# OpenMined/PIR

Measured on AMD Instinct MI355X. Metric: PIR queries/sec (ms/query in ms_per_step), N=4096 DB=2^20 x 288B d=2, higher is better.
Workload: dtype u64; 1 GPU; N=4096, 2 RNS data primes (36,36 bit | special 37 bit), t=24 bit, DB=2^20 x 288B, d=2, dims=[162, 162], num_pt=26215, 64 queries/step (whole job), 16 in flight per GPU (BASELINE.json configs[2]); workers=16, dist_mode=single, exchange=none, parallelism=single GPU, database_copies_in_hbm=operand layout only (u64 staging released)

## Files before the change

### pir_amd/build.py

```python
from __future__ import annotations

import os
import subprocess
import sys

HERE = os.path.dirname(os.path.abspath(__file__))
CSRC = os.path.join(HERE, "csrc")
LIB = os.path.join(HERE, "libpirgpu.so")
SOURCES = ["kernels.hip", "scan_mfma.hip", "ctx.hip", "wire.cpp", "wire_codec.cpp",
           "ntt_ring32k.hip",
           "ctmult.hip",
           "ctmult_rowsum.hip",
           "ctmult_shared.hip"]
NTT_SOURCE = "ntt_kernels.hip"
NTT_LOGNS = [11, 12, 13, 14]
NTT_PACK_BYTES = [5, 6, 7]
HEADERS = ["device_params.h", "env_gate.h", "options.h", "kernels.h", "host_math.h", "wire.h", "wire_codec.h", "arith.h", "ntt_core.h", "ctmult.h", "ctmult_convert.h", "scan_mfma_body.inc", NTT_SOURCE, os.path.join("..", "..", "include", "pirgpu.h")]
HIPCC = os.environ.get("HIPCC", "/opt/rocm/bin/hipcc")
FLAGS = ["--offload-arch=gfx950", "-O3", "-std=c++17", "-fPIC", "-Wall", "-Wno-unused-function"] + \
    os.environ.get("PIRGPU_BUILD_DEFS", "").split()


def ntt_object(logn: int, pb: int) -> str:
    return "ntt_kernels_%d.o" % logn if pb == 5 else "ntt_kernels_%d_p%d.o" % (logn, pb)


def _stale() -> bool:
    if not os.path.exists(LIB):
        return True
    t = os.path.getmtime(LIB)
    for f in SOURCES + HEADERS + [os.path.basename(__file__)]:
        p = os.path.join(CSRC, f) if f != os.path.basename(__file__) else os.path.join(HERE, f)
        if os.path.exists(p) and os.path.getmtime(p) > t:
            return True
    return False


def build(force: bool = False, verbose: bool = False) -> str:
    if not force and not _stale():
        return LIB
    jobs = []
    for src in SOURCES:
# ... 50 lines not shown
```

### pir_amd/csrc/ctx.hip

```cpp
#include <hip/hip_runtime.h>
#include <ctype.h>
#include <stdint.h>
#include <stdio.h>
#include <stdlib.h>
#include <string.h>

#include <algorithm>
#include <atomic>
#include <functional>
#include <map>
#include <mutex>
#include <string>
#include <vector>

#include "../../include/pirgpu.h"
#include "ctmult.h"
#include "device_params.h"
#include "host_math.h"
#include "kernels.h"
#include "options.h"
#include "wire.h"

using namespace pirgpu;

// ... 38 lines not shown
  uint32_t keyset = 0;
  uint32_t table = 0;
  uint64_t *res_a = nullptr, *res_b = nullptr, *prod = nullptr, *dig = nullptr, *sv_ntt = nullptr;
  uint64_t* d_query = nullptr;
  uint32_t staged_nq = 0;
  const uint64_t* sv_cur = nullptr;
  const uint64_t* sv_rows = nullptr;
  std::vector<uint64_t*> lvl;
  uint64_t* last = nullptr;
  uint64_t* pt_buf = nullptr;
  uint64_t* scan_part = nullptr;
  uint64_t* up_scratch = nullptr;
  size_t up_scratch_words = 0;
  uint8_t* selp = nullptr;
  bool reply_valid = false;
  hipEvent_t ev_expanded = nullptr, ev_scanned = nullptr;
  hipEvent_t ev_done = nullptr;
  hipEvent_t ev_join = nullptr;
};

struct HeadSlot {
  uint64_t *res_a = nullptr, *res_b = nullptr, *dig = nullptr, *prod = nullptr;
  hipEvent_t ev_ready = nullptr;
  hipEvent_t ev_free = nullptr;
  bool in_use = false;
};

struct BatchLane {
  hipStream_t stream = nullptr;
  HeadSlot head[2];
  uint32_t head_next = 0;
  uint64_t *res_a = nullptr, *res_b = nullptr, *prod = nullptr, *dig = nullptr;
  uint8_t* selp = nullptr;
  uint8_t* selp_runs = nullptr;
  hipEvent_t ev_scanned = nullptr;
  hipEvent_t ev_join = nullptr;
  std::vector<uint64_t*> lvl;
  uint64_t* last = nullptr;
  uint64_t* pt_buf = nullptr;
  uint64_t* scan_part = nullptr;
  uint64_t* up_scratch = nullptr;
  size_t up_scratch_words = 0;
};

struct Stage {
  hipStream_t stream;
  uint64_t* const* lvl;
  uint64_t* pt_buf;
  uint32_t n;
  MfmaPtrs sel;
  bool local_rows;
  uint64_t** up_scratch = nullptr;
  size_t* up_scratch_words = nullptr;
  bool sel_f64 = false;
  uint64_t* last = nullptr;
  bool rows_inverted = false;
  uint32_t ksets[kMaxMfmaQueries] = {};
};

struct CtmScratch {
  uint64_t* buf = nullptr;
  size_t words = 0;
  uint64_t* selc = nullptr;
  size_t selc_words = 0;
  uint64_t* selb = nullptr;
};
// ... 85 lines not shown
  std::map<uint32_t, uint16_t*> gperm;

  bool ws_ready = false;
  std::vector<Worker> workers;
  std::vector<uint64_t> lvl_rows;
  std::vector<uint64_t> lvl_cts;
  uint64_t m_max = 1;
  uint64_t pt_words = 0;
  BatchSet sets[kBatchSets];
  BatchSet& bs();
  uint32_t n_active = 1;
  uint32_t upper_blocks = 0;
  uint32_t upper_blocks_batch = 0;
  uint32_t scan_wgs_batch = 0;
  int64_t slots_scan_wgs = -1;
  bool slots_gather_ntt = false, slots_blk_major = false;
  bool tables_one_launch = false;
  int64_t ctm_rowsum_splits = 0;
  bool in_batch = false;
  uint32_t scan_nsplit = 1, scan_cps = 0, scan_rows = 0, scan_cols = 0;
  uint32_t scan_rpt = 0, scan_block = 0;
  bool scan_limb = false;
  uint32_t mq_nq = 4, mq_rows = 1;
  bool mq_single = false;
  uint32_t mq_single_rows = 4;
  bool mq_single_limb = false;
  uint64_t scan_npt = 0;
  bool mfma_on = false;
  MfmaGeom mg{};
  uint32_t mfma_nq = 0;
  bool mfma_single = false;
  bool scan_f64_fold = false;
  bool scan_f64_fold_batch = false;
  bool split_upper = false;
  uint64_t split_upper_words = 0;
  bool loop_transforms = false;
  uint32_t loop_min_sources = 1024;
  uint32_t fuse_mac_nodes = 128;
  bool fuse_mac_combine = false;
  bool fuse_last_level = false;
  bool last_level_ntt = false;
  bool tree40 = false;
  bool c0_ntt = false;
  bool c0_ntt_split = false;
  bool want_sel_f64 = false;
  bool sel_f64 = false;
  bool pack40 = false;
  int pack_bytes = 5;
  uint8_t* d_dbp = nullptr;
  bool packed_valid = false;
  bool staging_released = false;
  bool streamed = false;
  uint64_t stream_bands = 1;
  uint64_t db_bytes = 0, dbp_alloc = 0, mem_scratch = 0, mem_peak = 0;
  std::vector<BatchLane> lanes;
  uint64_t groups_run = 0;
  hipStream_t head_stream = nullptr;
  uint32_t head_levels = 0;
  uint32_t head_mode = 0;
  hipEvent_t ev_head_tail = nullptr;
  hipStream_t copy_stream = nullptr;
  hipEvent_t ev_fetch[2] = {nullptr, nullptr};
  hipEvent_t ev_fork = nullptr;
  hipEvent_t ev_main_join = nullptr;

  bool ctm = false;
// ... 354 lines not shown
  if (c->logN >= 15) c->split_upper = true;
  c->split_upper_words = (uint64_t)opt_u32(c, OPT_SPLIT_UPPER_MB, 3072) * (1ull << 20) / 8;
  c->loop_transforms = opt_u32(c, OPT_LOOP_TRANSFORMS, 1) != 0 && c->mode != kNttInt;
  c->pack40 = opt_u32(c, OPT_PACK40, 1) != 0;
  {
    uint32_t bits = 0;
    for (uint32_t j = 0; j <= k; ++j) bits = std::max<uint32_t>(bits, 64 - (uint32_t)__builtin_clzll(c->hp.mod[j].q));
    const int need = bits <= 39 ? 5 : (bits <= 47 ? 6 : (bits <= 55 ? 7 : 8));
    int want = (int)opt_u32(c, OPT_PACK_BYTES, (uint32_t)need);
    if (want < need) want = need;
    if (c->mode == kNttInt && want != 5) want = 8;
    if (c->logN >= 15) want = 8;
    if (want > 7) c->pack40 = false;
    c->pack_bytes = c->pack40 ? want : 5;
    if (c->pack40 && c->pack_bytes == 7 && c->logN >= 14 && !opt_u32(c, OPT_TREE40_WIDE, 0)) c->tree40 = false;
    const NttOps* ops = ntt_ops_for(N, c->pack_bytes);
    if (ops != c->ops) {
      c->ops = ops;
      HIP_TRY(c->ops->configure(c->mode));
    }
  }
  bool wide_given = false;
  const int64_t wide = c->options.value(OPT_SCAN_MFMA_WIDE, 0, &wide_given);
  c->mg = mfma_geometry(c->hp, c->scan_rows, c->scan_cols, wide_given ? (int)(wide != 0) : -1,
                        opt_u32(c, OPT_SCAN_MFMA_TOP4, 1) != 0);
  c->mfma_on = opt_u32(c, OPT_SCAN_MFMA, 1) != 0 && d >= 2 && c->mg.L != 0 && c->scan_rows >= 8 && c->scan_npt > 0;
  if (c->slot_sharded && (!c->mfma_on || c->mg.nchunks != 1 || c->nslots % c->mg.NW))
    throw Fail{PIRGPU_INVALID_ARGUMENT, "a slot shard needs the int8-MFMA scan in one column chunk (d = 2, >= 8 rows, "
                                        "moduli below 2^55, at most 28 column groups)"};
  c->mfma_nq = std::max<uint32_t>(1, std::min<uint32_t>(opt_u32(c, OPT_SCAN_MFMA_NQ, kMaxMfmaQueries), kMaxMfmaQueries));
  c->mfma_single = opt_u32(c, OPT_SCAN_MFMA_SINGLE, c->mg.nchunks == 1 ? 1 : 0) != 0;
  c->scan_f64_fold = opt_u32(c, OPT_SCAN_F64_FOLD, c->mg.L >= 6 ? 1 : 0) != 0;
  c->scan_f64_fold_batch = opt_u32(c, OPT_SCAN_F64_FOLD_BATCH, 1) != 0;
  for (uint32_t j = 0; j < k; ++j) {
    c->scan_f64_fold = c->scan_f64_fold && (c->hp.mod[j].q >> 50) == 0;
    c->scan_f64_fold_batch = c->scan_f64_fold_batch && (c->hp.mod[j].q >> 50) == 0;
  }
  const uint64_t rem = c->dim_sum % N;
  c->sel_f64 = c->want_sel_f64 && c->mfma_on && c->mode != kNttInt && c->fuse_last_level && c->last_level_ntt &&
               !c->split_upper && c->dim_sum >= 2 && rem != 1 && !c->ctm;
  if (c->ctm) c->ctm_scratch_words = (uint64_t)std::max<int64_t>(1, c->options.value(OPT_CT_SCRATCH_MB, 256)) * (1ull << 20) / 8;
  c->ctm_shared_sel = c->ctm && c->options.value(OPT_CT_SHARED_SEL, ctm_shared_sel_default(c)) != 0;
  if (c->streamed && c->mfma_on) {
    const uint64_t mb = (uint64_t)std::max<int64_t>(0, c->options.value(OPT_DB_STREAM_MB, 256));
    c->stream_bands = std::min<uint64_t>(std::max<uint64_t>(1, (mb << 20) / stream_band_bytes(c)), 65535);
    c->mfma_single = true;
  }
}

void ensure_workspace(pirgpu_ctx* c) {
  if (c->ws_ready) return;
  const uint32_t N = c->N, k = c->k, d = c->d;

  const uint64_t m_max = std::min<uint64_t>(N, hm::next_power_two(std::max<uint32_t>(c->dim_sum, 1)));
  c->m_max = m_max;
  const uint64_t shard_pts = matrix_pts(c);
  if (d == 1) {
    c->scan_rows = c->planes;
    c->scan_cols = (uint32_t)(shard_pts / c->planes);
  } else {
    c->scan_cols = c->dims[d - 1];
    c->scan_rows = (uint32_t)ceil_div(shard_pts, c->scan_cols);
  }
  c->scan_npt = shard_pts;
  resolve_options(c);
  c->lvl_rows.assign(d, 0);
// ... 398 lines not shown
  const uint64_t words = (uint64_t)c->scan_rows * c->ctw;
  ensure_packed(c);
  uint64_t* const out = c->mg.nchunks > 1 ? part : out_base;
  const uint64_t out_qstride = c->mg.nchunks > 1 ? (uint64_t)c->mg.nchunks * words : words;
  if (!packed) {
    if (!selp) selp = c->dalloc<uint8_t>(c->mg.sel_bytes);
    HIP_TRY(launch_sel_pack(st, c->dp, c->mg, col_sel, n, selp, c->scan_cols, kN, sel_f64));
    packed = selp;
  }
  if (profiled) record(c, *profiled, PH_SCAN);
  const bool share = share_chip && !profiled && c->scan_wgs_batch;
  const uint32_t wgs = share ? c->scan_wgs_batch : 0;
  constexpr uint32_t kMaxBscan = 64;
  const bool timed = c->prof && !profiled && c->bscan_n < kMaxBscan;
  if (timed) {
    while (c->bscan_ev.size() < 2 * (size_t)(c->bscan_n + 1)) {
      hipEvent_t e;
      HIP_TRY(hipEventCreate(&e));
      c->bscan_ev.push_back(e);
    }
    HIP_TRY(hipEventRecord(c->bscan_ev[2 * c->bscan_n], st));
  }
  HIP_TRY(launch_scan_mfma(st, c->dp, c->mg, table_dbp(c, table), packed, out, out_qstride, n, c->scan_rows, kN, words, wgs,
                           n > 1 ? (c->scan_f64_fold || c->scan_f64_fold_batch) : c->scan_f64_fold));
  if (!profiled) ++c->options.counter(OPT_SCAN_LAUNCHES);
  if (timed) {
    HIP_TRY(hipEventRecord(c->bscan_ev[2 * c->bscan_n + 1], st));
    ++c->bscan_n;
    c->bscan_wgs = wgs;
    c->bscan_nq = n;
  }
  if (c->mg.nchunks > 1)
    HIP_TRY(launch_reduce_splits(st, c->dp, part, c->mg.nchunks, words, out_base, n, (uint64_t)c->mg.nchunks * words, words));
}

void scan_on_device(pirgpu_ctx* c, Worker& w) {
  const uint32_t N = c->N, k = c->k;
  const size_t ctw = c->ctw;
  refuse_slot_shard(c);
  if (!table_loaded(c, w.table))
    throw Fail{PIRGPU_FAILED_PRECONDITION, c->tables > 1 ? "table " + std::to_string(w.table) + " not fully loaded"
                                                         : std::string("database not fully loaded")};
  check_transparent(c, w.table);
  if (c->pt_end == c->pt_begin) return;
  if (c->mfma_on && c->mfma_single) {
    MfmaPtrs col{};
    col.p[0] = scan_selectors(c, w);
    scan_group_mfma(c, w.stream, w.selp, col, 1, scan_out(c, w), w.scan_part, &w, nullptr, false, false, w.table);
    return;
  }
  const uint64_t* sv_base = scan_selectors(c, w);
  uint64_t* base_out = scan_out(c, w);
  const uint64_t* db = table_db(c, w.table);
  if (c->mq_single && mq_usable(c)) {
    HIP_TRY(launch_scan_mq(w.stream, c->dp, N, k, db, &sv_base, &base_out, 1, c->scan_rows, c->scan_cols,
                           c->mq_single_rows, c->mq_single_limb && c->scan_limb));
    return;
  }
  uint64_t* scan_out = c->scan_nsplit > 1 ? w.scan_part : base_out;
  HIP_TRY(launch_scan(w.stream, c->dp, N, k, db, sv_base, scan_out, c->scan_rows, c->scan_cols, c->scan_npt,
                      c->scan_nsplit, c->scan_cps, c->scan_rpt, c->scan_block, c->scan_limb));
  if (c->scan_nsplit > 1)
    HIP_TRY(launch_reduce_splits(w.stream, c->dp, w.scan_part, c->scan_nsplit, (uint64_t)c->scan_rows * ctw,
                                 base_out));
}

// ... 2107 lines not shown
}

static void ensure_lanes(pirgpu_ctx* c, bool with_expansion_buffers) {
  const uint32_t N = c->N, k = c->k;
  if (c->lanes.empty()) {
    const uint32_t n_lanes = 2;
    c->lanes.resize(n_lanes);
    for (BatchLane& ln : c->lanes) {
      HIP_TRY(hipStreamCreateWithFlags(&ln.stream, hipStreamNonBlocking));
      HIP_TRY(hipEventCreateWithFlags(&ln.ev_scanned, hipEventDisableTiming));
    }
  }
  if (with_expansion_buffers && !c->lanes[0].res_a) {
    const uint64_t half = std::max<uint64_t>(c->m_max / 2, 1);
    for (BatchLane& ln : c->lanes) {
      ln.res_a = c->dalloc<uint64_t>((size_t)kMaxMfmaQueries * c->m_max * c->ctw);
      ln.res_b = c->dalloc<uint64_t>((size_t)kMaxMfmaQueries * c->m_max * c->ctw);
      ln.prod = c->dalloc<uint64_t>((size_t)kMaxMfmaQueries * half * 2 * (k + 1) * N);
      ln.dig = c->dalloc<uint64_t>((size_t)kMaxMfmaQueries * half * (k + 1) * k * N);
    }
  }
  if (c->mfma_on && c->lanes[0].lvl.empty()) {
    for (BatchLane& ln : c->lanes) {
      ln.lvl.assign(c->d, nullptr);
      for (uint32_t l = 0; l < c->d; ++l) ln.lvl[l] = c->dalloc<uint64_t>((size_t)kMaxMfmaQueries * c->lvl_cts[l] * c->ctw);
      if (c->rp) ln.last = c->dalloc<uint64_t>((size_t)kMaxMfmaQueries * c->lvl_cts[0] * c->ctw);
      if (c->pt_words) ln.pt_buf = c->dalloc<uint64_t>((size_t)kMaxMfmaQueries * c->pt_words);
      if (c->mg.nchunks > 1)
        ln.scan_part = c->dalloc<uint64_t>((size_t)kMaxMfmaQueries * c->mg.nchunks * std::max<uint32_t>(c->scan_rows, 1) * c->ctw);
    }
  }
}

static void ensure_head_slot(pirgpu_ctx* c, HeadSlot& hs) {
  if (hs.res_a) return;
  const uint32_t N = c->N, k = c->k;
  const uint64_t cts = ((uint64_t)1 << c->head_levels) * kMaxMfmaQueries;
  hs.res_a = c->dalloc<uint64_t>(cts * c->ctw);
  hs.res_b = c->dalloc<uint64_t>(cts * c->ctw);
  hs.prod = c->dalloc<uint64_t>(std::max<uint64_t>(cts / 2, 1) * 2 * (k + 1) * N);
  hs.dig = c->dalloc<uint64_t>(std::max<uint64_t>(cts / 2, 1) * (k + 1) * k * N);
  HIP_TRY(hipEventCreateWithFlags(&hs.ev_ready, hipEventDisableTiming));
  HIP_TRY(hipEventCreateWithFlags(&hs.ev_free, hipEventDisableTiming));
  if (!c->head_stream) {
    HIP_TRY(hipStreamCreateWithFlags(&c->head_stream, hipStreamNonBlocking));
    HIP_TRY(hipEventCreateWithFlags(&c->ev_head_tail, hipEventDisableTiming));
  }
}

static void expand_group_on_lane(pirgpu_ctx* c, BatchLane& ln, Worker* const* members, uint32_t B, uint32_t first,
                                 bool sel_f64 = false, uint64_t* sv_dst = nullptr, const uint32_t* qidx = nullptr) {
  const uint32_t N = c->N, k = c->k;
  const uint32_t nq = c->dim_sum / N + 1;
  const size_t ctw = c->ctw, qwords = (size_t)nq * ctw;
  uint64_t remaining = c->dim_sum, produced = 0;
  const bool use_head = nq == 1 && B > 1 && c->head_levels > 0 && (c->head_mode == 2 || (c->head_mode == 1 && c->bs().st_pieces > 0)) &&
                        hm::ceil_log2((uint32_t)std::min<uint64_t>(c->dim_sum, N)) >= c->head_levels + 2;
  const uint32_t ws_first = qidx ? 0 : first, ws_n = qidx ? c->bs().staged_count : B;
  if (!use_head) wait_staged(c, ln.stream, ws_first, ws_n);
  auto import_roots = [&](hipStream_t st, uint64_t* dst, uint32_t qc) {
    if (!qidx) {
      HIP_TRY(launch_tree_convert(st, c->dp, c->mode, c->bs().d_bquery + (size_t)first * qwords + (size_t)qc * ctw, dst,
                                  (uint64_t)B * ctw, true, ctw, qwords));
      return;
    }
    for (uint32_t q = 0; q < B; ++q)
// ... 103 lines not shown
}

static uint32_t lanes_in_use(pirgpu_ctx* c, uint32_t G) {
  const uint32_t W = std::max<uint32_t>(1, std::min<uint32_t>(c->n_active, (uint32_t)c->workers.size()));
  return std::max<uint32_t>(1, std::min<uint32_t>((uint32_t)c->lanes.size(), W / std::max<uint32_t>(G, 1)));
}

static void batch_run_mfma(pirgpu_ctx* c, uint32_t count, const uint64_t* ext_sv, const PackedInput* pk = nullptr,
                           const uint32_t* qtab = nullptr) {
  const size_t rwords = (size_t)c->reply_cts * c->rctw, svwords = (size_t)c->dim_sum * c->ctw;
  const uint32_t W = std::max<uint32_t>(1, std::min<uint32_t>(c->n_active, (uint32_t)c->workers.size()));
  const uint32_t G = std::min<uint32_t>(c->mfma_nq, W);
  TablePlan tp;
  if (qtab) tp = plan_table_runs(qtab, count, G);
  const uint32_t* order = qtab && !tp.identity ? tp.order.data() : nullptr;
  auto oq = [&](uint32_t pos) { return order ? order[pos] : pos; };
  auto tab = [&](uint32_t pos) { return qtab ? qtab[oq(pos)] : 0u; };
  std::vector<uint8_t> done(order ? count : 0, 0);
  uint32_t lead = 0;
  const uint32_t my_rows = c->se - c->sb;
  ensure_lanes(c, !ext_sv && !pk);
  const uint32_t nl = lanes_in_use(c, G);
  const uint32_t span = pk ? pk->per_rank : count;
  uint32_t n_groups = 0;
  for (uint32_t rank0 = 0; rank0 < count; rank0 += span) {
    const uint32_t in_span = std::min<uint32_t>(span, count - rank0);
    n_groups += (in_span + (pk ? (uint32_t)kMaxMfmaQueries : G) - 1) / (pk ? (uint32_t)kMaxMfmaQueries : G);
  }
  const bool share_chip = n_groups >= 2 && nl >= 2;
  const bool host_dl = c->bs().host_reply && (uint64_t)count * c->reply_cts <= c->bs().host_reply_cts;
  c->bs().host_reply_done = host_dl;
  c->bs().dl_end.clear();
  c->bs().dl_next = 0;
  for (uint32_t rank0 = 0; rank0 < count; rank0 += span) {
    const uint32_t step = pk ? (uint32_t)kMaxMfmaQueries : G;
    const uint32_t in_span = std::min<uint32_t>(span, count - rank0);
    for (uint32_t j0 = 0; j0 < in_span; j0 += step) {
      const uint32_t B = std::min<uint32_t>(step, in_span - j0);
      if (B > W) throw Fail{PIRGPU_FAILED_PRECONDITION, "packed groups need min(queries per rank, 8) workers (pirgpu_set_concurrency)"};
      const uint32_t li = (uint32_t)(c->groups_run++ % nl);
      BatchLane& ln = c->lanes[li];
      Worker* members[kMaxMfmaQueries];
      for (uint32_t q = 0; q < B; ++q) {
        members[q] = &c->workers[(li * G + q) % W];
        HIP_TRY(hipStreamWaitEvent(ln.stream, members[q]->ev_done, 0));
      }
      const uint32_t first = rank0 + j0;
      const uint8_t* packed = nullptr;
      uint64_t* lvl_ptrs[PIRGPU_MAX_DIMS];
      for (uint32_t l = 0; l < c->d; ++l) lvl_ptrs[l] = ln.lvl[l];
      const bool direct_reply = c->d >= 2 && !order;
      if (direct_reply) lvl_ptrs[0] = reply_base(c) + (size_t)first * rwords;
      Stage sg{ln.stream, lvl_ptrs, ln.pt_buf, B, MfmaPtrs{}, pk != nullptr, &ln.up_scratch, &ln.up_scratch_words};
      sg.last = ln.last;
      for (uint32_t q = 0; q < B; ++q)
        sg.ksets[q] = oq(first + q) < c->bs().batch_keysets.size() ? c->bs().batch_keysets[oq(first + q)] : 0;
      MfmaPtrs col{};
      if (pk) {
        const uint32_t groups_per_rank = (pk->per_rank + kMaxMfmaQueries - 1) / kMaxMfmaQueries;
        packed = pk->packed + ((size_t)(rank0 / pk->per_rank) * groups_per_rank + j0 / kMaxMfmaQueries) * c->mg.sel_bytes;
        for (uint32_t q = 0; q < B; ++q) sg.sel.p[q] = pk->rows + (size_t)(first + q) * my_rows * c->ctw;
      } else {
        if (!ext_sv) {
          expand_group_on_lane(c, ln, members, B, first, c->sel_f64, nullptr, order ? order + first : nullptr);
          sg.sel_f64 = c->sel_f64;
        }
        for (uint32_t q = 0; q < B; ++q) {
          const uint64_t* sv = ext_sv ? ext_sv + (size_t)oq(first + q) * svwords : members[q]->sv_ntt;
          sg.sel.p[q] = sv;
          col.p[q] = sv + (size_t)c->sv_off[c->d - 1] * c->ctw;
        }
      }
      uint32_t rb[kMaxMfmaQueries + 1], tabs[kMaxMfmaQueries], nr = 0;
      for (uint32_t q = 0; q < B; ++q)
        if (q == 0 || tab(first + q) != tab(first + q - 1)) {
          rb[nr] = q;
          tabs[nr++] = tab(first + q);
        }
      rb[nr] = B;
      if (nr == 1)
        scan_group_mfma(c, ln.stream, ln.selp, col, B, ln.lvl[c->d - 1], ln.scan_part, nullptr, packed, sg.sel_f64,
                        share_chip, tabs[0]);
      else
        scan_group_runs(c, ln, col, B, rb, nr, tabs, sg.sel_f64, share_chip);
      post_scan_stage(c, sg, nullptr);
      if (order) {
        for (uint32_t q = 0; q < B; ++q)
          HIP_TRY(hipMemcpyAsync(reply_base(c) + (size_t)oq(first + q) * rwords, ln.lvl[0] + (size_t)q * rwords, rwords * 8,
                                 hipMemcpyDeviceToDevice, ln.stream));
      } else if (!direct_reply)
        HIP_TRY(hipMemcpyAsync(reply_base(c) + (size_t)first * rwords, ln.lvl[0], (size_t)B * rwords * 8,
                               hipMemcpyDeviceToDevice, ln.stream));
      if (host_dl) {
        BatchSet& b = c->bs();
        const size_t gi = b.dl_end.size();
        while (gi >= b.dl_events.size()) {
          hipEvent_t e;
          HIP_TRY(hipEventCreateWithFlags(&e, hipEventDisableTiming));
          b.dl_events.push_back(e);
          HIP_TRY(hipEventCreateWithFlags(&e, hipEventDisableTiming));
          b.rd_events.push_back(e);
        }
        if (!c->copy_stream) HIP_TRY(hipStreamCreateWithFlags(&c->copy_stream, hipStreamNonBlocking));
        HIP_TRY(hipEventRecord(b.rd_events[gi], ln.stream));
        HIP_TRY(hipStreamWaitEvent(c->copy_stream, b.rd_events[gi], 0));
        if (order) {
          for (uint32_t q = 0; q < B; ++q) {
            const size_t at = (size_t)oq(first + q) * rwords;
            HIP_TRY(hipMemcpyAsync(b.host_reply + at, reply_base(c) + at, rwords * 8, hipMemcpyDeviceToHost, c->copy_stream));
            done[oq(first + q)] = 1;
          }
          while (lead < count && done[lead]) ++lead;
        } else {
          HIP_TRY(hipMemcpyAsync(b.host_reply + (size_t)first * rwords, reply_base(c) + (size_t)first * rwords,
                                 (size_t)B * rwords * 8, hipMemcpyDeviceToHost, c->copy_stream));
        }
        HIP_TRY(hipEventRecord(b.dl_events[gi], c->copy_stream));
        b.dl_end.push_back(order ? lead : first + B);
      }
      for (uint32_t q = 0; q < B; ++q) {
        HIP_TRY(hipEventRecord(members[q]->ev_done, ln.stream));
        members[q]->reply_valid = false;
      }
    }
  }
}

static void batch_run_impl_body(pirgpu_ctx* c, uint32_t count, const uint64_t* ext_sv);
static void batch_run_impl(pirgpu_ctx* c, uint32_t count, const uint64_t* ext_sv) {
  struct Flag {
    bool& f;
    explicit Flag(bool& x) : f(x) { f = true; }
    ~Flag() { f = false; }
  } flag(c->in_batch);
  batch_run_impl_body(c, count, ext_sv);
}
static void batch_run_impl_body(pirgpu_ctx* c, uint32_t count, const uint64_t* ext_sv) {
  refuse_slot_shard(c);
  c->bs().host_reply_done = false;
  const size_t rwords = (size_t)c->reply_cts * c->rctw;
  const size_t svwords = (size_t)c->dim_sum * c->ctw;
  const uint32_t W = std::max<uint32_t>(1, std::min<uint32_t>(c->n_active, (uint32_t)c->workers.size()));
  const uint32_t G = mq_usable(c) && c->pt_end > c->pt_begin ? std::min<uint32_t>(c->mq_nq, kMaxScanQueries) : 1;
  std::vector<uint32_t> qtab_v;
  if (c->tables > 1) {
    qtab_v = c->bs().batch_tables.size() == count ? c->bs().batch_tables : std::vector<uint32_t>(count, c->cur_table);
    for (uint32_t t : qtab_v) {
      if (!table_loaded(c, t)) throw Fail{PIRGPU_FAILED_PRECONDITION, "table " + std::to_string(t) + " not fully loaded"};
      check_transparent(c, t);
    }
  } else {
// ... 636 lines not shown
```

### pir_amd/csrc/kernels.h

```cpp
#pragma once
#include <hip/hip_runtime.h>
#include <stdint.h>

#include "device_params.h"

namespace pirgpu {

constexpr int kMaxScanChunks = 16;
constexpr int kMaxMfmaQueries = 8;
constexpr int kMaxScanGroups = 16;
constexpr int kMaxSlices = 16;

constexpr uint32_t kKsWideLevel = 256;
inline bool ks_digit_takes_c0(uint32_t nodes) { return nodes >= kKsWideLevel && nodes % 8 == 0; }

struct MfmaPtrs {
  const void* p[kMaxMfmaQueries];
};

struct ScanGroups {
  uint32_t n;
  const uint8_t* sel[kMaxScanGroups];
  uint64_t* out[kMaxScanGroups];
  uint8_t nq[kMaxScanGroups];
// ... 111 lines not shown
  uint32_t GC;
  uint32_t nchunks;
  uint32_t NW;
  uint32_t top4;
  uint32_t tile_bytes;
  size_t db_bytes, sel_bytes;
};

MfmaGeom mfma_geometry(const DevParams& hp, uint32_t rows, uint32_t cols, int wide_override = -1, bool allow_top4 = true);
hipError_t launch_db_pack(hipStream_t st, const DevParams* P, const MfmaGeom& gm, const uint64_t* db, uint8_t* dbp,
                          uint32_t rows, uint32_t cols, uint32_t kN, uint32_t slot0 = 0, uint32_t nslots = 0);
hipError_t launch_db_pack_band(hipStream_t st, const DevParams* P, const MfmaGeom& gm, const uint64_t* band, uint8_t* dbp,
                               uint32_t rt0, uint32_t n_rt, uint64_t npts, uint32_t cols, uint32_t kN, uint32_t slot0 = 0,
                               uint32_t nslots = 0);
hipError_t launch_db_unpack(hipStream_t st, const DevParams* P, const MfmaGeom& gm, const uint8_t* dbp, uint64_t* out,
                            uint32_t row, uint32_t col, uint32_t kN);
struct DbUnit {
  uint32_t r, kg, mask, out0;
};
hipError_t launch_db_gather(hipStream_t st, const DevParams* P, const MfmaGeom& gm, const uint8_t* dbp,
                            const DbUnit* units, uint32_t n_units, uint64_t* out, uint32_t N);
hipError_t launch_db_pack_update(hipStream_t st, const DevParams* P, const MfmaGeom& gm, const uint64_t* enc,
                                 const DbUnit* units, uint32_t n_units, uint8_t* dbp, uint32_t kN, uint32_t slot0,
                                 uint32_t nslots);
hipError_t launch_sel_pack(hipStream_t st, const DevParams* P, const MfmaGeom& gm, const MfmaPtrs& sv, uint32_t nq,
                           uint8_t* selp, uint32_t cols, uint32_t kN, bool sel_f64 = false, const SliceMap* map = nullptr);
hipError_t launch_scan_mfma(hipStream_t st, const DevParams* P, const MfmaGeom& gm, const uint8_t* dbp,
                            const uint8_t* selp, uint64_t* out, uint64_t out_qstride, uint32_t nq, uint32_t rows,
                            uint32_t kN, uint64_t chunk_stride, uint32_t wgs = 0, bool f64_fold = false);
hipError_t launch_scan_mfma_groups(hipStream_t st, const DevParams* P, const MfmaGeom& gm, const uint8_t* dbp,
                                   const ScanGroups& grp, uint32_t rows, uint64_t chunk_stride, uint32_t wgs, bool f64_fold,
                                   uint32_t slot0, uint32_t nslots, uint64_t out_qstride, uint32_t out_rstride,
                                   bool blk_major = false);
bool scan_mfma_runs_supported(const MfmaGeom& gm);
hipError_t launch_scan_mfma_runs(hipStream_t st, const DevParams* P, const MfmaGeom& gm, const ScanGroupsDb& grp,
                                 uint32_t rows, uint32_t kN, uint64_t chunk_stride, uint32_t wgs, bool f64_fold,
                                 uint64_t out_qstride);
hipError_t launch_slots_assemble(hipStream_t st, const uint64_t* src, uint64_t* dst, const SliceMap& map, uint32_t RC,
                                 uint32_t kN, uint32_t nq, uint64_t dst_qstride, uint32_t nq_total, uint32_t q0);

}
```

Baseline: 5492 queries/s.

## Add paired-group MFMA scan kernel reusing each database tile across two query groups

Adds a new MFMA scan kernel that multiplies every loaded database tile against the selectors of two query groups (16 queries) before moving on. The group-1 selector is kept in registers and the group-2 selector is staged in LDS. The batch loop now pairs consecutive groups, expanding both on one lane, running the paired scan, then running the post-scan stages and downloads for each half. This roughly halves database HBM traffic per query, which matters because the scan is bandwidth-bound. In exchange it uses more LDS and registers, allocates extra per-lane buffers, and serializes two groups on one lane, which reduces overlap across streams.

```diff
diff --git a/pir_amd/build.py b/pir_amd/build.py
--- a/pir_amd/build.py
+++ b/pir_amd/build.py
@@ -7,7 +7,7 @@
 HERE = os.path.dirname(os.path.abspath(__file__))
 CSRC = os.path.join(HERE, "csrc")
 LIB = os.path.join(HERE, "libpirgpu.so")
-SOURCES = ["kernels.hip", "scan_mfma.hip", "ctx.hip", "wire.cpp", "wire_codec.cpp",
+SOURCES = ["kernels.hip", "scan_mfma.hip", "scan_mfma_pair.hip", "ctx.hip", "wire.cpp", "wire_codec.cpp",
            "ntt_ring32k.hip",
            "ctmult.hip",
            "ctmult_rowsum.hip",
diff --git a/pir_amd/csrc/ctx.hip b/pir_amd/csrc/ctx.hip
--- a/pir_amd/csrc/ctx.hip
+++ b/pir_amd/csrc/ctx.hip
@@ -94,6 +94,9 @@
   uint32_t head_next = 0;
   uint64_t *res_a = nullptr, *res_b = nullptr, *prod = nullptr, *dig = nullptr;
   uint8_t* selp = nullptr;
+  uint64_t* sv2 = nullptr;
+  uint8_t* selp2 = nullptr;
+  uint64_t* rows2 = nullptr;
   uint8_t* selp_runs = nullptr;
   hipEvent_t ev_scanned = nullptr;
   hipEvent_t ev_join = nullptr;
@@ -245,6 +248,7 @@
   bool mfma_single = false;
   bool scan_f64_fold = false;
   bool scan_f64_fold_batch = false;
+  uint32_t scan_pair = 1;
   bool split_upper = false;
   uint64_t split_upper_words = 0;
   bool loop_transforms = false;
@@ -665,6 +669,9 @@
   c->mfma_single = opt_u32(c, OPT_SCAN_MFMA_SINGLE, c->mg.nchunks == 1 ? 1 : 0) != 0;
   c->scan_f64_fold = opt_u32(c, OPT_SCAN_F64_FOLD, c->mg.L >= 6 ? 1 : 0) != 0;
   c->scan_f64_fold_batch = opt_u32(c, OPT_SCAN_F64_FOLD_BATCH, 1) != 0;
+  c->scan_pair = 1;
+  if (const char* v = pirgpu_env("PIRGPU_SCAN_MFMA_PAIR"))
+    if (*v) c->scan_pair = (uint32_t)std::min<long>(2, std::max<long>(0, strtol(v, nullptr, 10)));
   for (uint32_t j = 0; j < k; ++j) {
     c->scan_f64_fold = c->scan_f64_fold && (c->hp.mod[j].q >> 50) == 0;
     c->scan_f64_fold_batch = c->scan_f64_fold_batch && (c->hp.mod[j].q >> 50) == 0;
@@ -1129,6 +1136,43 @@
   }
   if (c->mg.nchunks > 1)
     HIP_TRY(launch_reduce_splits(st, c->dp, part, c->mg.nchunks, words, out_base, n, (uint64_t)c->mg.nchunks * words, words));
+}
+
+static void scan_pair_mfma(pirgpu_ctx* c, BatchLane& ln, const MfmaPtrs (&col)[2], const uint32_t (&n)[2],
+                           uint64_t* const (&out)[2], bool sel_f64, bool share_chip) {
+  const uint32_t kN = c->k * c->N;
+  const uint64_t words = (uint64_t)c->scan_rows * c->ctw;
+  hipStream_t st = ln.stream;
+  ensure_packed(c);
+  if (!ln.selp) ln.selp = c->dalloc<uint8_t>(c->mg.sel_bytes);
+  uint8_t* const selp[2] = {ln.selp, ln.selp2};
+  ScanGroups grp{};
+  grp.n = 2;
+  for (uint32_t h = 0; h < 2; ++h) {
+    HIP_TRY(launch_sel_pack(st, c->dp, c->mg, col[h], n[h], selp[h], c->scan_cols, kN, sel_f64));
+    grp.sel[h] = selp[h];
+    grp.out[h] = out[h];
+    grp.nq[h] = (uint8_t)n[h];
+  }
+  const uint32_t wgs = share_chip && c->scan_wgs_batch ? c->scan_wgs_batch : 0;
+  const bool timed = c->prof && c->bscan_n < 64;
+  if (timed) {
+    while (c->bscan_ev.size() < 2 * (size_t)(c->bscan_n + 1)) {
+      hipEvent_t e;
+      HIP_TRY(hipEventCreate(&e));
+      c->bscan_ev.push_back(e);
+    }
+    HIP_TRY(hipEventRecord(c->bscan_ev[2 * c->bscan_n], st));
+  }
+  HIP_TRY(launch_scan_mfma_pair(st, c->dp, c->mg, c->d_dbp, grp, c->scan_rows, words, wgs,
+                                c->scan_f64_fold || c->scan_f64_fold_batch, 0, kN, words, kN));
+  ++c->options.counter(OPT_SCAN_LAUNCHES);
+  if (timed) {
+    HIP_TRY(hipEventRecord(c->bscan_ev[2 * c->bscan_n + 1], st));
+    ++c->bscan_n;
+    c->bscan_wgs = wgs;
+    c->bscan_nq = n[0] + n[1];
+  }
 }
 
 void scan_on_device(pirgpu_ctx* c, Worker& w) {
@@ -3302,6 +3346,13 @@
   }
 }
 
+static void ensure_pair_buffers(pirgpu_ctx* c, BatchLane& ln, bool expands) {
+  if (expands && !ln.sv2) ln.sv2 = c->dalloc<uint64_t>((size_t)kMaxMfmaQueries * c->dim_sum * c->ctw);
+  if (ln.selp2) return;
+  ln.selp2 = c->dalloc<uint8_t>(c->mg.sel_bytes);
+  ln.rows2 = c->dalloc<uint64_t>((size_t)kMaxMfmaQueries * c->lvl_cts[c->d - 1] * c->ctw);
+}
+
 static void ensure_head_slot(pirgpu_ctx* c, HeadSlot& hs) {
   if (hs.res_a) return;
   const uint32_t N = c->N, k = c->k;
@@ -3471,11 +3522,77 @@
   c->bs().host_reply_done = host_dl;
   c->bs().dl_end.clear();
   c->bs().dl_next = 0;
+  auto queue_download = [&](BatchLane& ln, uint32_t first, uint32_t B) {
+    BatchSet& b = c->bs();
+    const size_t gi = b.dl_end.size();
+    while (gi >= b.dl_events.size()) {
+      hipEvent_t e;
+      HIP_TRY(hipEventCreateWithFlags(&e, hipEventDisableTiming));
+      b.dl_events.push_back(e);
+      HIP_TRY(hipEventCreateWithFlags(&e, hipEventDisableTiming));
+      b.rd_events.push_back(e);
+    }
+    if (!c->copy_stream) HIP_TRY(hipStreamCreateWithFlags(&c->copy_stream, hipStreamNonBlocking));
+    HIP_TRY(hipEventRecord(b.rd_events[gi], ln.stream));
+    HIP_TRY(hipStreamWaitEvent(c->copy_stream, b.rd_events[gi], 0));
+    HIP_TRY(hipMemcpyAsync(b.host_reply + (size_t)first * rwords, reply_base(c) + (size_t)first * rwords,
+                           (size_t)B * rwords * 8, hipMemcpyDeviceToHost, c->copy_stream));
+    HIP_TRY(hipEventRecord(b.dl_events[gi], c->copy_stream));
+    b.dl_end.push_back(first + B);
+  };
+  const bool may_pair = c->scan_pair && !pk && !qtab && c->d >= 2 && !c->ctm && !c->rp && c->planes <= 1 &&
+                        G == (uint32_t)kMaxMfmaQueries && scan_mfma_pair_supported(c->mg) &&
+                        (c->scan_pair >= 2 || (n_groups >= 4 && nl >= 2));
+  auto run_pair = [&](uint32_t first_a, uint32_t Ba, uint32_t first_b, uint32_t Bb) {
+    const uint32_t li = (uint32_t)(c->groups_run++ % nl);
+    BatchLane& ln = c->lanes[li];
+    ensure_pair_buffers(c, ln, !ext_sv);
+    const bool sel_f64 = !ext_sv && c->sel_f64;
+    Worker* members[kMaxMfmaQueries];
+    for (uint32_t q = 0; q < Ba; ++q) {
+      members[q] = &c->workers[(li * G + q) % W];
+      HIP_TRY(hipStreamWaitEvent(ln.stream, members[q]->ev_done, 0));
+    }
+    if (!ext_sv) {
+      expand_group_on_lane(c, ln, members, Ba, first_a, sel_f64);
+      expand_group_on_lane(c, ln, members, Bb, first_b, sel_f64, ln.sv2);
+    }
+    const uint32_t firsts[2] = {first_a, first_b}, n[2] = {Ba, Bb};
+    uint64_t* const rows_out[2] = {ln.lvl[c->d - 1], ln.rows2};
+    MfmaPtrs sel[2] = {}, col[2] = {};
+    for (uint32_t h = 0; h < 2; ++h)
+      for (uint32_t q = 0; q < n[h]; ++q) {
+        sel[h].p[q] = ext_sv ? ext_sv + (size_t)(firsts[h] + q) * svwords : (h ? ln.sv2 + (size_t)q * svwords : members[q]->sv_ntt);
+        col[h].p[q] = (const uint64_t*)sel[h].p[q] + (size_t)c->sv_off[c->d - 1] * c->ctw;
+      }
+    scan_pair_mfma(c, ln, col, n, rows_out, sel_f64, share_chip);
+    for (uint32_t h = 0; h < 2; ++h) {
+      uint64_t* lvl_ptrs[PIRGPU_MAX_DIMS];
+      for (uint32_t l = 0; l < c->d; ++l) lvl_ptrs[l] = ln.lvl[l];
+      lvl_ptrs[c->d - 1] = rows_out[h];
+      lvl_ptrs[0] = reply_base(c) + (size_t)firsts[h] * rwords;
+      Stage sg{ln.stream, lvl_ptrs, ln.pt_buf, n[h], sel[h], false, &ln.up_scratch, &ln.up_scratch_words};
+      sg.sel_f64 = sel_f64;
+      for (uint32_t q = 0; q < n[h]; ++q)
+        sg.ksets[q] = firsts[h] + q < c->bs().batch_keysets.size() ? c->bs().batch_keysets[firsts[h] + q] : 0;
+      post_scan_stage(c, sg, nullptr);
+      if (host_dl) queue_download(ln, firsts[h], n[h]);
+    }
+    for (uint32_t q = 0; q < Ba; ++q) {
+      HIP_TRY(hipEventRecord(members[q]->ev_done, ln.stream));
+      members[q]->reply_valid = false;
+    }
+  };
   for (uint32_t rank0 = 0; rank0 < count; rank0 += span) {
     const uint32_t step = pk ? (uint32_t)kMaxMfmaQueries : G;
     const uint32_t in_span = std::min<uint32_t>(span, count - rank0);
     for (uint32_t j0 = 0; j0 < in_span; j0 += step) {
       const uint32_t B = std::min<uint32_t>(step, in_span - j0);
+      if (may_pair && j0 + step < in_span) {
+        run_pair(rank0 + j0, B, rank0 + j0 + step, std::min<uint32_t>(step, in_span - j0 - step));
+        j0 += step;
+        continue;
+      }
       if (B > W) throw Fail{PIRGPU_FAILED_PRECONDITION, "packed groups need min(queries per rank, 8) workers (pirgpu_set_concurrency)"};
       const uint32_t li = (uint32_t)(c->groups_run++ % nl);
       BatchLane& ln = c->lanes[li];
@@ -3531,31 +3648,30 @@
         HIP_TRY(hipMemcpyAsync(reply_base(c) + (size_t)first * rwords, ln.lvl[0], (size_t)B * rwords * 8,
                                hipMemcpyDeviceToDevice, ln.stream));
       if (host_dl) {
-        BatchSet& b = c->bs();
-        const size_t gi = b.dl_end.size();
-        while (gi >= b.dl_events.size()) {
-          hipEvent_t e;
-          HIP_TRY(hipEventCreateWithFlags(&e, hipEventDisableTiming));
-          b.dl_events.push_back(e);
-          HIP_TRY(hipEventCreateWithFlags(&e, hipEventDisableTiming));
-          b.rd_events.push_back(e);
-        }
-        if (!c->copy_stream) HIP_TRY(hipStreamCreateWithFlags(&c->copy_stream, hipStreamNonBlocking));
-        HIP_TRY(hipEventRecord(b.rd_events[gi], ln.stream));
-        HIP_TRY(hipStreamWaitEvent(c->copy_stream, b.rd_events[gi], 0));
-        if (order) {
+        if (!order) {
+          queue_download(ln, first, B);
+        } else {
+          BatchSet& b = c->bs();
+          const size_t gi = b.dl_end.size();
+          while (gi >= b.dl_events.size()) {
+            hipEvent_t e;
+            HIP_TRY(hipEventCreateWithFlags(&e, hipEventDisableTiming));
+            b.dl_events.push_back(e);
+            HIP_TRY(hipEventCreateWithFlags(&e, hipEventDisableTiming));
+            b.rd_events.push_back(e);
+          }
+          if (!c->copy_stream) HIP_TRY(hipStreamCreateWithFlags(&c->copy_stream, hipStreamNonBlocking));
+          HIP_TRY(hipEventRecord(b.rd_events[gi], ln.stream));
+          HIP_TRY(hipStreamWaitEvent(c->copy_stream, b.rd_events[gi], 0));
           for (uint32_t q = 0; q < B; ++q) {
             const size_t at = (size_t)oq(first + q) * rwords;
             HIP_TRY(hipMemcpyAsync(b.host_reply + at, reply_base(c) + at, rwords * 8, hipMemcpyDeviceToHost, c->copy_stream));
             done[oq(first + q)] = 1;
           }
           while (lead < count && done[lead]) ++lead;
-        } else {
-          HIP_TRY(hipMemcpyAsync(b.host_reply + (size_t)first * rwords, reply_base(c) + (size_t)first * rwords,
-                                 (size_t)B * rwords * 8, hipMemcpyDeviceToHost, c->copy_stream));
+          HIP_TRY(hipEventRecord(b.dl_events[gi], c->copy_stream));
+          b.dl_end.push_back(lead);
         }
-        HIP_TRY(hipEventRecord(b.dl_events[gi], c->copy_stream));
-        b.dl_end.push_back(order ? lead : first + B);
       }
       for (uint32_t q = 0; q < B; ++q) {
         HIP_TRY(hipEventRecord(members[q]->ev_done, ln.stream));
diff --git a/pir_amd/csrc/kernels.h b/pir_amd/csrc/kernels.h
--- a/pir_amd/csrc/kernels.h
+++ b/pir_amd/csrc/kernels.h
@@ -167,6 +167,11 @@
                                    const ScanGroups& grp, uint32_t rows, uint64_t chunk_stride, uint32_t wgs, bool f64_fold,
                                    uint32_t slot0, uint32_t nslots, uint64_t out_qstride, uint32_t out_rstride,
                                    bool blk_major = false);
+bool scan_mfma_pair_supported(const MfmaGeom& gm);
+hipError_t launch_scan_mfma_pair(hipStream_t st, const DevParams* P, const MfmaGeom& gm, const uint8_t* dbp,
+                                 const ScanGroups& grp, uint32_t rows, uint64_t chunk_stride, uint32_t wgs, bool f64_fold,
+                                 uint32_t slot0, uint32_t nslots, uint64_t out_qstride, uint32_t out_rstride,
+                                 bool blk_major = false);
 bool scan_mfma_runs_supported(const MfmaGeom& gm);
 hipError_t launch_scan_mfma_runs(hipStream_t st, const DevParams* P, const MfmaGeom& gm, const ScanGroupsDb& grp,
                                  uint32_t rows, uint32_t kN, uint64_t chunk_stride, uint32_t wgs, bool f64_fold,
diff --git a/pir_amd/csrc/scan_mfma_pair.hip b/pir_amd/csrc/scan_mfma_pair.hip
--- /dev/null
+++ b/pir_amd/csrc/scan_mfma_pair.hip
@@ -0,0 +1,302 @@
+#include <hip/hip_runtime.h>
+
+#include <stdlib.h>
+
+#include <algorithm>
+
+#include "arith.h"
+#include "kernels.h"
+
+namespace pirgpu {
+
+namespace {
+
+typedef int v4i __attribute__((ext_vector_type(4)));
+typedef int v2i __attribute__((ext_vector_type(2)));
+
+__host__ __device__ __forceinline__ constexpr uint32_t pair_tile_bytes(uint32_t L, bool top4) {
+  return top4 ? (L - 1) * 256 + 128 : L * 256;
+}
+__device__ __forceinline__ uint32_t pair_sx4(uint32_t v) { return v | (((v >> 3) & 0x01010101u) * 0xF0u); }
+__device__ __forceinline__ v4i pair_expand_top4(v2i w) {
+  const uint32_t w0 = (uint32_t)w[0], w1 = (uint32_t)w[1];
+  return v4i{(int)pair_sx4(w0 & 0x0F0F0F0Fu), (int)pair_sx4((w0 >> 4) & 0x0F0F0F0Fu), (int)pair_sx4(w1 & 0x0F0F0F0Fu),
+              (int)pair_sx4((w1 >> 4) & 0x0F0F0F0Fu)};
+}
+__device__ __forceinline__ v4i pair_load_tile(const uint8_t* p) {
+  return __builtin_nontemporal_load(reinterpret_cast<const v4i*>(p));
+}
+__device__ __forceinline__ v2i pair_load_tile8(const uint8_t* p) {
+  return __builtin_nontemporal_load(reinterpret_cast<const v2i*>(p));
+}
+constexpr int kPairBiasBits = 59;
+
+}
+
+template <int L, int KS, bool TOP4, bool F64F>
+__global__ void __launch_bounds__(512)
+scan_mfma_pair_kernel(const DevParams* __restrict__ P, const uint8_t* __restrict__ dbp, ScanGroups grp, uint32_t rows,
+                      uint32_t RT, uint32_t KG, uint32_t nslots, uint64_t out_qstride) {
+  constexpr int NW = 8;
+  constexpr uint32_t TB = pair_tile_bytes(L, TOP4);
+  constexpr int LF = TOP4 ? L - 1 : L;
+  constexpr int NS = 2 * L - 1;
+  constexpr int NG = (NS + 4) / 5;
+  __shared__ __attribute__((aligned(16))) uint64_t stage[2][16][16][NW + 1];
+  __shared__ __attribute__((aligned(16))) v4i selb[NW][KS * L][64];
+  const int w = __builtin_amdgcn_readfirstlane((int)(threadIdx.x >> 6)), l = threadIdx.x & 63;
+  const int g = l >> 4, i16 = l & 15;
+  const uint32_t nunits = nslots >> 3;
+  const size_t slab = (size_t)RT * KG * TB;
+  const size_t rt_stride = (size_t)KG * TB;
+  const uint32_t lane16 = i16 * 16, lane8 = i16 * 8;
+  v4i* const myb = &selb[w][0][l];
+
+  v4i B[KS][L], A[KS][LF];
+  v2i A4[KS];
+  auto load_B = [&](uint32_t gi, uint32_t jl) __attribute__((always_inline)) {
+    const uint8_t* selp = grp.sel[gi];
+    const uint32_t nx = 2u * grp.nq[gi];
+#pragma unroll
+    for (int ks = 0; ks < KS; ++ks) {
+      const uint32_t kg = ks * 4 + g;
+      const uint8_t* blk = selp + ((size_t)jl * KG + kg) * TB;
+#pragma unroll
+      for (int b = 0; b < L; ++b) {
+        B[ks][b] = v4i{0, 0, 0, 0};
+        if (kg < KG && (uint32_t)i16 < nx) {
+          if (TOP4 && b == L - 1) B[ks][b] = pair_expand_top4(*reinterpret_cast<const v2i*>(blk + b * 256 + lane8));
+          else B[ks][b] = *reinterpret_cast<const v4i*>(blk + b * 256 + lane16);
+        }
+      }
+    }
+  };
+  v4i N[LF];
+  v2i N4;
+  auto load_N = [&](uint32_t gi, uint32_t jl, int ks) __attribute__((always_inline)) {
+    const uint8_t* selp = grp.sel[gi];
+    const uint32_t nx = 2u * grp.nq[gi];
+    const uint32_t kg = ks * 4 + g;
+    const uint8_t* blk = selp + ((size_t)jl * KG + kg) * TB;
+    const bool in = kg < KG && (uint32_t)i16 < nx;
+#pragma unroll
+    for (int b = 0; b < LF; ++b) {
+      N[b] = v4i{0, 0, 0, 0};
+      if (in) N[b] = *reinterpret_cast<const v4i*>(blk + b * 256 + lane16);
+    }
+    N4 = v2i{0, 0};
+    if (TOP4 && in) N4 = *reinterpret_cast<const v2i*>(blk + (L - 1) * 256 + lane8);
+  };
+  auto store_N = [&](int ks) __attribute__((always_inline)) {
+#pragma unroll
+    for (int b = 0; b < LF; ++b) myb[(ks * L + b) * 64] = N[b];
+    if constexpr (TOP4) myb[(ks * L + L - 1) * 64] = pair_expand_top4(N4);
+  };
+  auto load_A = [&](int ks, const uint8_t* base, uint32_t kg) __attribute__((always_inline)) {
+    const uint8_t* blk = base + (size_t)kg * TB;
+#pragma unroll
+    for (int a = 0; a < LF; ++a) A[ks][a] = pair_load_tile(blk + a * 256 + lane16);
+    if constexpr (TOP4) A4[ks] = pair_load_tile8(blk + (L - 1) * 256 + lane8);
+  };
+
+  uint32_t u = blockIdx.x;
+  if (u >= nunits) return;
+  {
+    const uint32_t blk = u;
+    load_B(0, blk * NW + w);
+    const uint8_t* abase = dbp + (size_t)(blk * NW + w) * slab;
+#pragma unroll
+    for (int ks = 0; ks < KS; ++ks) {
+      const uint32_t kg = ks * 4 + g;
+#pragma unroll
+      for (int a = 0; a < LF; ++a) A[ks][a] = v4i{0, 0, 0, 0};
+      A4[ks] = v2i{0, 0};
+      if (kg < KG) load_A(ks, abase, kg);
+    }
+#pragma unroll
+    for (int ks = 0; ks < KS; ++ks) {
+      load_N(1, blk * NW + w, ks);
+      store_N(ks);
+    }
+  }
+
+  for (; u < nunits; u += gridDim.x) {
+    const uint32_t j0 = u * NW;
+    const uint32_t mi = (j0 + w) >> P->logN;
+    const ModConst m = P->mod[mi];
+    const uint64_t bias = m.q << (kPairBiasBits - (64 - __builtin_clzll(m.q)));
+    [[maybe_unused]] const F64Mod fm{P->tab[mi].qd, P->tab[mi].qinvd};
+    [[maybe_unused]] const double fw0 = P->fold_w[mi][0], fw1 = P->fold_w[mi][1], fw2 = P->fold_w[mi][2];
+    const uint8_t* abase = dbp + (size_t)(j0 + w) * slab;
+    const uint32_t nu = u + gridDim.x;
+    const bool has_next = nu < nunits;
+    const uint32_t nblk = has_next ? nu : u;
+    const uint8_t* nbase = dbp + (size_t)(nblk * NW + w) * slab;
+
+    auto fold = [&](v4i (&T)[NS], int buf) __attribute__((always_inline)) {
+#pragma unroll
+      for (int i = 0; i < 4; ++i) {
+        uint64_t r = 0;
+        if constexpr (F64F) {
+          constexpr int NC = (NS + 3) / 4;
+          double acc = 0.0;
+#pragma unroll
+          for (int c = NC - 1; c >= 0; --c) {
+            double C = 0.0;
+#pragma unroll
+            for (int s = (4 * c + 3 < NS ? 4 * c + 3 : NS - 1); s >= 4 * c; --s) C = __builtin_fma(C, 256.0, (double)T[s][i]);
+            if (c == 0) acc += f64_norm(C, fm);
+            else acc += f64_mulmod(C, c == 1 ? fw0 : (c == 2 ? fw1 : fw2), fm);
+          }
+          r = f64_to_u64(f64_canon(f64_norm(acc, fm), fm));
+        } else {
+#pragma unroll
+          for (int gq = NG - 1; gq >= 0; --gq) {
+            int64_t G = 0;
+#pragma unroll
+            for (int s = gq * 5; s < gq * 5 + 5 && s < NS; ++s) G += (int64_t)T[s][i] << (8 * (s - gq * 5));
+            if (gq == NG - 1 && NG > 1) {
+              r = (uint64_t)(G + (int64_t)bias);
+            } else {
+              const u128 v = ((u128)r << 40) + (uint64_t)(G + (int64_t)bias);
+              r = reduce128((uint64_t)v, (uint64_t)(v >> 64), m);
+            }
+          }
+        }
+        stage[buf][g * 4 + i][i16][w] = r;
+      }
+    };
+    auto store = [&](int buf, uint32_t rt, uint32_t nx, uint64_t* obase) __attribute__((always_inline)) {
+      __syncthreads();
+#pragma unroll
+      for (int round = 0; round < 2; ++round) {
+        const int run = round * 128 + (threadIdx.x >> 2);
+        const int part = threadIdx.x & 3;
+        const int r16 = run >> 4, x = run & 15;
+        const uint32_t r = rt * 16 + r16;
+        if (x < (int)nx && r < rows) {
+          typedef unsigned long long ull2 __attribute__((ext_vector_type(2)));
+          const ull2 v = {stage[buf][r16][x][part * 2], stage[buf][r16][x][part * 2 + 1]};
+          uint64_t* dst = obase + (size_t)(x >> 1) * out_qstride + ((size_t)r * 2 + (x & 1)) * nslots + j0 + part * 2;
+          *reinterpret_cast<ull2*>(dst) = v;
+        }
+      }
+    };
+    const uint32_t nx0 = 2u * grp.nq[0], nx1 = 2u * grp.nq[1];
+    uint64_t* const obase0 = grp.out[0];
+    uint64_t* const obase1 = grp.out[1];
+
+    for (uint32_t rt = 0; rt < RT; ++rt) {
+      v4i T[NS];
+      const bool last = rt + 1 == RT;
+      const uint8_t* next_tile = last ? nbase : abase + (size_t)(rt + 1) * rt_stride;
+      const bool refill = !last || has_next;
+      const bool next_sel = last && has_next;
+
+#pragma unroll
+      for (int s = 0; s < NS; ++s) T[s] = v4i{0, 0, 0, 0};
+#pragma unroll
+      for (int ks = 0; ks < KS; ++ks) {
+        [[maybe_unused]] v4i Atop;
+        if constexpr (TOP4) Atop = pair_expand_top4(A4[ks]);
+#pragma unroll
+        for (int off = 0; off < L; ++off)
+#pragma unroll
+          for (int a = 0; a < L; ++a) {
+            const int b = (a + off) % L;
+            if (TOP4 && a == L - 1)
+              T[a + b] = __builtin_amdgcn_mfma_i32_16x16x64_i8(Atop, B[ks][b], T[a + b], 0, 0, 0);
+            else
+              T[a + b] = __builtin_amdgcn_mfma_i32_16x16x64_i8(A[ks][a < LF ? a : 0], B[ks][b], T[a + b], 0, 0, 0);
+          }
+      }
+      if (next_sel) load_B(0, nblk * NW + w);
+      fold(T, 0);
+      store(0, rt, nx0, obase0);
+
+#pragma unroll
+      for (int s = 0; s < NS; ++s) T[s] = v4i{0, 0, 0, 0};
+#pragma unroll
+      for (int ks = 0; ks < KS; ++ks) {
+        [[maybe_unused]] v4i Atop;
+        if constexpr (TOP4) Atop = pair_expand_top4(A4[ks]);
+#pragma unroll
+        for (int b = 0; b < L; ++b) {
+          const v4i Bt = myb[(ks * L + b) * 64];
+#pragma unroll
+          for (int a = 0; a < L; ++a) {
+            if (TOP4 && a == L - 1) T[a + b] = __builtin_amdgcn_mfma_i32_16x16x64_i8(Atop, Bt, T[a + b], 0, 0, 0);
+            else T[a + b] = __builtin_amdgcn_mfma_i32_16x16x64_i8(A[ks][a < LF ? a : 0], Bt, T[a + b], 0, 0, 0);
+          }
+        }
+        if (next_sel) {
+          if (ks > 0) store_N(ks - 1);
+          if (ks < KS - 1) load_N(1, nblk * NW + w, ks);
+        }
+        const uint32_t kg = ks * 4 + g;
+        if (refill && kg < KG) load_A(ks, next_tile, kg);
+      }
+      fold(T, 1);
+      if (next_sel) load_N(1, nblk * NW + w, KS - 1);
+      store(1, rt, nx1, obase1);
+      if (next_sel) store_N(KS - 1);
+    }
+  }
+}
+
+
+static uint32_t scan_pair_wgs_all() {
+  static const uint32_t wgs_all = [] {
+    const char* v = pirgpu_env("PIRGPU_SCAN_MFMA_WGS");
+    if (v && *v) return (uint32_t)strtoul(v, nullptr, 10);
+    hipDeviceProp_t prop;
+    int dev = 0;
+    if (hipGetDevice(&dev) != hipSuccess || hipGetDeviceProperties(&prop, dev) != hipSuccess) return 256u;
+    return (uint32_t)prop.multiProcessorCount;
+  }();
+  return wgs_all;
+}
+
+bool scan_mfma_pair_supported(const MfmaGeom& gm) {
+  return gm.L == 5 && gm.NW == 8 && gm.nchunks == 1 && gm.KS >= 1 && gm.KS <= 3;
+}
+
+template <int L, int KS, bool TOP4, bool F64F>
+static void launch_scan_mfma_pair_variant(hipStream_t st, const DevParams* P, const MfmaGeom& gm, const uint8_t* dbp,
+                                          const ScanGroups& grp, uint32_t rows, uint32_t wgs_req, uint32_t nslots,
+                                          uint64_t out_qstride) {
+  const uint32_t all = scan_pair_wgs_all();
+  const uint32_t wgs = wgs_req ? std::min(wgs_req, all) : all;
+  const uint32_t units = nslots / 8;
+  hipLaunchKernelGGL((scan_mfma_pair_kernel<L, KS, TOP4, F64F>), dim3(std::max(1u, std::min(units, wgs))), dim3(512), 0, st,
+                     P, dbp, grp, rows, gm.RT, gm.KG, nslots, out_qstride);
+}
+
+hipError_t launch_scan_mfma_pair(hipStream_t st, const DevParams* P, const MfmaGeom& gm, const uint8_t* dbp,
+                                 const ScanGroups& grp, uint32_t rows, uint64_t chunk_stride, uint32_t wgs, bool f64_fold,
+                                 uint32_t slot0, uint32_t nslots, uint64_t out_qstride, uint32_t out_rstride, bool blk_major) {
+  (void)chunk_stride;
+  if (!scan_mfma_pair_supported(gm) || grp.n != 2 || slot0 != 0 ||
+      nslots == 0 || nslots % 8 || out_rstride != nslots || blk_major)
+    return hipErrorInvalidValue;
+  for (uint32_t g = 0; g < grp.n; ++g)
+    if (!grp.sel[g] || !grp.out[g] || grp.nq[g] == 0 || grp.nq[g] > kMaxMfmaQueries) return hipErrorInvalidValue;
+#define PIRGPU_PAIR_ARGS st, P, gm, dbp, grp, rows, wgs, nslots, out_qstride
+#define PIRGPU_PAIR_CASE(KS_)                                                            \
+  if (gm.KS == KS_) {                                                                    \
+    if (gm.top4) {                                                                       \
+      if (f64_fold) launch_scan_mfma_pair_variant<5, KS_, true, true>(PIRGPU_PAIR_ARGS); \
+      else launch_scan_mfma_pair_variant<5, KS_, true, false>(PIRGPU_PAIR_ARGS);         \
+    } else {                                                                             \
+      if (f64_fold) launch_scan_mfma_pair_variant<5, KS_, false, true>(PIRGPU_PAIR_ARGS); \
+      else launch_scan_mfma_pair_variant<5, KS_, false, false>(PIRGPU_PAIR_ARGS);        \
+    }                                                                                    \
+    return hipGetLastError();                                                            \
+  }
+  PIRGPU_PAIR_CASE(1) PIRGPU_PAIR_CASE(2) PIRGPU_PAIR_CASE(3)
+#undef PIRGPU_PAIR_CASE
+#undef PIRGPU_PAIR_ARGS
+  return hipErrorInvalidValue;
+}
+
+}
```

After: 5672 queries/s (median of 6 runs). 3.3% higher.
